# bowang-lab/gcn-drug-repurposing

Measured on AMD Instinct MI355X. Metric: gcn_spmm_edges_per_s, higher is better.
Workload: dtype f32; 1 GPU; whole_graph stand-in (value = 2.001e+10 edges/s counts every SpMM at nnz as the reference executes it; value_executed = 1.69e+10 counts the entries the kernels visited): N=29960, nnz(A_hat)=988028, d=128, L=2, B=2048, 15 steps/epoch; full train step (fwd+gss_loss+bwd+Adam), 6 SpMMs/step counted at nnz each (algorithmic; the top layer's first backward SpMM visits only entries whose neighbour is a b; parallelism=single; nodes relabelled hub-first

## Files before the change

gcn-drug-repurposing_amd/_lib.py:

```python
from __future__ import annotations

import ctypes as C
import os
import subprocess

_HERE = os.path.dirname(os.path.abspath(__file__))
LIB_PATH = os.path.join(_HERE, "libgssgcn.so")
CSRC = os.path.join(_HERE, "csrc")
ABI_VERSION = 21

_lib = None


class GssError(RuntimeError):
    pass


class PlanDesc(C.Structure):
    _fields_ = [("n", C.c_int32), ("d", C.c_int32), ("num_layers", C.c_int32), ("max_batch", C.c_int32),
                ("layer_decay", C.c_float), ("alpha", C.c_float), ("lr", C.c_float), ("beta1", C.c_float),
                ("beta2", C.c_float), ("eps", C.c_float), ("cache_layer1", C.c_int32), ("pipeline_layer1", C.c_int32),
                ("node_map", C.c_void_p)]


# ... 91 lines not shown
    "gss_edgelist_bad_line": (_I64, [_P]),
    "gss_edgelist_copy": (C.c_int, [_P, _P, _P, _P]),
    "gss_edgelist_close": (None, [_P]),
    "gss_plan_create": (C.c_int, [C.POINTER(_P), C.POINTER(PlanDesc), _P, _P, C.POINTER(PlanIO)]),
    "gss_plan_create_sharded": (C.c_int, [C.POINTER(_P), C.POINTER(PlanDesc), C.POINTER(ShardDesc), _P, _P, _P, C.POINTER(PlanIO)]),
    "gss_plan_gather_embeddings": (C.c_int, [_P, _P, _P]),
    "gss_plan_destroy": (None, [_P]),
    "gss_plan_forward": (C.c_int, [_P, _P]),
    "gss_plan_loss_backward": (C.c_int, [_P, _P, _I32, _F, _P]),
    "gss_plan_backward": (C.c_int, [_P, _P, _I32, _P, _P]),
    "gss_plan_adam": (C.c_int, [_P, _P]),
    "gss_plan_step": (C.c_int, [_P, _P, _I32, _F, _P]),
    "gss_plan_step_lazy": (C.c_int, [_P, _P, _I32, _F, _P]),
    "gss_plan_activation": (_P, [_P, C.c_int, C.c_int]),
    "gss_plan_device_bytes": (_SZ, [_P]),
    "gss_plan_check_guards": (C.c_int, [_P]),
    "gss_plan_lazy_halo_rows": (C.c_int, [_P, C.POINTER(_I64)]),
    "gss_plan_comm_stats": (C.c_int, [_P, C.POINTER(_I64)]),
    "gss_plan_sync_stats": (C.c_int, [_P, C.POINTER(_I64)]),
    "gss_comm_local_mode": (C.c_int, [_P, _I32]),
    "gss_comm_local_log": (C.c_int, [_P, C.POINTER(_I64), _I32, C.POINTER(_I32)]),
    "gss_plan_set_step": (None, [_P, _I32]),
    "gss_plan_adam_buffer": (_P, [_P, _I32, _I32]),
    "gss_plan_get_step": (_I32, [_P]),
    "gss_plan_profile": (C.c_int, [_P, C.c_int]),
    "gss_plan_profile_read": (C.c_int, [_P, C.POINTER(C.c_double), C.POINTER(C.c_int64), _P]),
    "gss_debug_set_option": (C.c_int, [C.c_char_p, C.c_int]),
    "gss_plan_debug_set_option": (C.c_int, [_P, C.c_char_p, C.c_int]),
    "gss_memcpy_d2d": (C.c_int, [_P, _P, _SZ, _P]),
    "gss_ppr_create": (C.c_int, [C.POINTER(_P), C.POINTER(PprDesc)]),
# ... 26 lines not shown
    "gss_rank_metrics_workspace_bytes": (_SZ, [_I32, _I32]),
    "gss_rank_metrics_rows": (C.c_int, [_I32, _I32, _P, _I64, _P, _P, _I32, _P, _P, _P, _P, _P, _P, _P, _SZ, _P]),
    "gss_profile_dist": (C.c_int, [_I32, _P, _I64, _I32, _P, _I32, _P, _I32, _P, _I64, _P]),
    "gss_profile_dist_pairs_workspace_bytes": (_SZ, [_I32, _I32]),
    "gss_profile_dist_pairs": (C.c_int, [_I32, _P, _I64, _I32, _P, _P, _I32, _P, _P, _SZ, _P]),
    "gss_profile_rank_workspace_bytes": (_SZ, [_I32, _I32]),
    "gss_profile_rank": (C.c_int, [_I32, _P, _I64, _I32, _P, _P, _I64, _P, _SZ, _P]),
    "gss_profile_topk_workspace_bytes": (_SZ, [_I32, _I32, _I32, _I32]),
    "gss_profile_topk": (C.c_int, [_I32, _P, _I64, _I32, _P, _I32, _P, _I32, _P, _P, _P, _P, _SZ, _P]),
    "gss_topk_overlap": (C.c_int, [_I32, _I32, _I32, _P, _P, _I32, _P, _P, _P, _P]),
    "gss_embedding_scores": (C.c_int, [_I32, _I32, _P, _I64, _I32, _P, _I32, _P, _I32, _P, _I64, _P]),
    "gss_spmm_bwd1_sparse_ex": (C.c_int, [_P, _I32, _P, _P, _P, _P, _P, _P, _P, _P, _P, _P, _I32, _P, _P]),
    "gss_spmm_bwd2_sparse_res": (C.c_int, [_P, _I32, _P, _P, _P, _F, _P, _P, _P, _P, _P, _P, _I32, _P]),
    "gss_spmm_filtered": (C.c_int, [_P, _I32, _P, _P, _P, _P, _P, _P, _P, _P, _P]),
    "gss_mark_rows_and_neighbours": (C.c_int, [_P, _P, _I32, _P, _P]),
    "gss_batch_bits": (C.c_int, [_P, _I32, _P, _I32, _P]),
    "gss_bits_fill": (C.c_int, [_P, _I64, _I64, _P]),
    "gss_loss_workspace_bytes_parts": (_SZ, [_I32, _I32, _I32]),
    "gss_loss_step": (C.c_int, [_I32, _I32, _F, _F, _P, _P, _P, _P, _P, _P, _P, _P, _F, _P, _P, _P, _P, _P, _P, _I32, _P, _P, _P, C.POINTER(_I32)]),
    "gss_loss_slab_sweep": (C.c_int, [_I32, _I32, _F, _F, _P, _I32, _I32, _P, _P, _P]),
    "gss_loss_gather_rows": (C.c_int, [_I32, _P, _P, _P, _I32, _P, C.POINTER(_P), _P]),
    "gss_loss_gather_rows_mapped": (C.c_int, [_I32, _P, _P, _P, _I32, _I32, _P, _P, _P, _P, _I32, _P, C.POINTER(_P), _P]),
    "gss_loss_gather_batch": (C.c_int, [_I32, _P, _P, _P, _P, _P, _I32, _I32, _P, _P, _P, _P, _P, _I32, _P, _P]),
    "gss_dense_fwd_rows": (C.c_int, [_I32, _I32, _P, _P, _P, _P, _P, _P, _P, _F, _P, _P, _P, _I32, _P]),
    "gss_dense_fwd_first": (C.c_int, [_I32, _I32, _P, _P, _P, _P]),
    "gss_dense_fwd_split_available": (C.c_int, [_I32, _I32]),
    "gss_dense_fwd_norm": (C.c_int, [_I32, _I32, _P, _P, _P, _P, _P, _P, _P, _F, _P, _P, _P, _P, _P, _P, _I32, _P]),
    "gss_rownorm_fwd_rows": (C.c_int, [_I32, _I32, _P, _P, _P, _P, _P]),
    "gss_wgrad_slices": (C.c_int, [_I32, _I32]),
    "gss_wgrad_slices_max": (C.c_int, [_I32, _I32]),
# ... 103 lines not shown
```

gcn-drug-repurposing_amd/csrc/ops.h:

```cpp
#pragma once
#include <memory>
#include <vector>

#include "common.h"

struct gss_giant_rows;

struct gss_csr {
  int32_t n_rows = 0, n_cols = 0;
  int64_t nnz = 0;
  const int32_t *rowptr = nullptr, *col = nullptr;
  const float *val = nullptr;
  int32_t n_long = 0;
  int32_t *d_long_rows = nullptr;
  int32_t max_row = 0;
  int32_t hot_own = -1, hot_halo0 = 0, hot_halo1 = 0;
  int32_t seg_edges = 32;
  std::vector<int32_t> h_rowptr;
  bool by_items = false;
  std::vector<int32_t> item_row, item_first, item_len;
  struct Cache {
    int32_t *segs[5] = {};
    int32_t seg_blocks[5] = {};
    std::unique_ptr<gss_giant_rows> giant;
// ... 43 lines not shown
};
int csr_segments(const gss_csr *a, int gpw_log2, const int4 **out, int *n_blocks);
struct LiveHint {
  int64_t prev;
  explicit LiveHint(int64_t rows);
  ~LiveHint();
  LiveHint(const LiveHint &) = delete;
  LiveHint &operator=(const LiveHint &) = delete;
};
int spmm_fwd(const gss_csr *a, int32_t d, const float *x, float *y, const float *h, float *m, void *stream,
             const int32_t *row_pos = nullptr,
             const uint32_t *row_bits = nullptr,
             const float *y_in = nullptr,
             const uint32_t *gather_bits = nullptr,
             const BatchPrep *prep = nullptr);
int mark_rows_and_neighbours(const gss_csr *a, const int32_t *rows, int32_t b, uint32_t *bits, void *stream);
int spmm_bwd1(const gss_csr *at, int32_t d, const float *g_am, const float *g_ax, const float *x_in, const float *ax,
              float *u, float *t, void *stream, const float *y_in = nullptr);
int spmm_bwd2(const gss_csr *at, int32_t d, const float *u, const float *t, const float *p, float c, const float *res,
              float *dp, float *gx_out, void *stream, const float *y_in = nullptr,
              int32_t own_row_limit = 0);
int dense_fwd(int32_t n, int32_t d, const float *ax, const float *am, const float *w1, const float *b1, const float *w2,
              const float *b2, const float *p_prev, float decay, float *p, float *x_next, void *stream,
              const int32_t *row_list = nullptr,
              bool acc_in_p = false);
bool dense_fwd_split_available(int32_t n, int32_t d);
bool dense_fwd_split_auto(int32_t n, int32_t d);
int dense_fwd_first(int32_t n, int32_t d, const float *ax, const float *w1, float *acc, void *stream);
bool dense_fwd_norm_available(int32_t d);
int dense_fwd_norm(int32_t n, int32_t d, const float *ax, const float *am, const float *w1, const float *b1, const float *w2,
// ... 107 lines not shown
```

gcn-drug-repurposing_amd/csrc/plan.hip:

```cpp
#include <algorithm>
#include <chrono>
#include <thread>
#include <vector>

#include "ops.h"

struct gss_plan {
  gss::Knobs knobs;
  gss_plan_desc desc;
  const gss_csr *a, *at;
  const float *x;
  float *w1, *b1, *w2, *b2;
  char *slab;
  size_t slab_bytes;
  std::vector<float *> ax, am, p, xin;
  float *m_tmp, *x_last, *emb, *inv_den;
  float *g_ax, *g_am, *u, *t, *dp, *gx[2];
  float *de_b, *dx_b, *dp_b, *gax_b, *gam_b;
  int32_t *pos;
  uint32_t *posbits;
  std::vector<size_t> guard_off;
  uint32_t *needbits;
  bool needbits_valid = false;
  uint32_t *nzbits;
  float *w1t, *w2t;
  float *grad[4];
  float *adam_m[4], *adam_v[4];
  float *loss;
  void *loss_ws, *wgrad_ws;
  int32_t step;
  bool layer1_valid;
  hipStream_t side;
  hipEvent_t ev_main_ready, ev_side_done;
  std::vector<hipEvent_t> ev_split_go, ev_split_done;
  float *ax0[2], *am0[2], *m_side;
  int cur0;
  bool prefetched;
  bool wt_valid;
  int wg_total;
  bool prof_on;
  std::vector<hipEvent_t> ev;
  std::vector<int> ev_cls;
  size_t ev_used;
  double prof_ms[GSS_PROF_CLASSES];
  int64_t prof_cnt[GSS_PROF_CLASSES];
  gss_comm *comm;
  int P, rank;
  int lo;
  std::vector<int64_t> h_bounds;
  struct Halo {
    int64_t n_halo = 0, n_send = 0;
    std::vector<int64_t> recv_off, send_off;
    const int32_t *d_send_rows = nullptr;
  } halo_a, halo_t;
  size_t rows_a, rows_t;
  const int32_t *gid2op_t;
  float *sendbuf;
// ... 44 lines not shown
  gss_plan *p;
  hipStream_t st;
  size_t slot;
  bool on;
  ProfScope(gss_plan *plan, int cls, void *stream) : p(plan), st(as_stream(stream)), slot(0), on(plan->prof_on) {
    if (!on) return;
    if (p->ev_used * 2 + 2 > p->ev.size()) {
      hipEvent_t a, b;
      if (hipEventCreate(&a) != hipSuccess || hipEventCreate(&b) != hipSuccess) {
        on = false;
        return;
      }
      p->ev.push_back(a);
      p->ev.push_back(b);
      p->ev_cls.push_back(cls);
    }
    slot = p->ev_used++;
    p->ev_cls[slot] = cls;
    (void)hipEventRecord(p->ev[2 * slot], st);
  }
  ~ProfScope() {
    if (on) (void)hipEventRecord(p->ev[2 * slot + 1], st);
  }
};
#define PROF(cls) ProfScope prof_scope_##__LINE__(p, cls, stream)

constexpr size_t kGuardBytes = 256;
constexpr int kGuardByte = 0xA5;
struct Carver {
  size_t off = 0;
  char *base = nullptr;
  std::vector<size_t> *guards = nullptr;
  template <typename T>
  T *take(size_t count) {
    off = (off + 255) / 256 * 256;
    T *p = base ? reinterpret_cast<T *>(base + off) : nullptr;
    off += sizeof(T) * count;
    off = (off + 255) / 256 * 256;
    if (guards) guards->push_back(off);
    off += kGuardBytes;
// ... 222 lines not shown
  p->a = a;
  p->at = at;
  p->x = io->x;
  p->w1 = io->w1;
  p->b1 = io->b1;
  p->w2 = io->w2;
  p->b2 = io->b2;
  p->emb = io->emb;
  p->loss = io->loss;
  p->grad[0] = io->gw1;
  p->grad[1] = io->gb1;
  p->grad[2] = io->gw2;
  p->grad[3] = io->gb2;
  p->step = 0;
  p->layer1_valid = false;
  p->wt_valid = false;

  p->prof_on = false;
  p->ev_used = 0;
  for (int k = 0; k < GSS_PROF_CLASSES; ++k) {
    p->prof_ms[k] = 0.0;
    p->prof_cnt[k] = 0;
  }
  {
    const int knob = K().lazy_halo, knob_u = K().lazy_halo_u;
    const bool rccl = comm && comm->device_transport();
    p->lz.on = P > 1 && desc->num_layers > 1 && (knob == 1 || (knob < 0 && n_global >= 262144 && !rccl));
    p->lzt.on = p->lz.on && spmm_sparse_available() && (knob_u == 1 || (knob_u < 0 && (knob == 1 || !rccl)));
    auto word_offsets = [&](gss_plan::LazyHalo &z, const gss_plan::Halo &h) {
      if (!z.on) return;
// ... 335 lines not shown

int plan_forward_impl(gss_plan *p, void *stream, const int32_t *lazy_rows = nullptr, int32_t lazy_b = 0) {
  if (p) p->needbits_valid = false;
  GSS_REQUIRE(p, "plan_forward: null plan");
  const gss_plan_desc &D = p->desc;
  const int L = D.num_layers;
  bool have_l0 = false;
  if (p->prefetched) {
    GSS_HIP(hipStreamWaitEvent(as_stream(stream), p->ev_side_done, 0));
    p->prefetched = false;
    p->cur0 ^= 1;
    p->ax[0] = p->ax0[p->cur0];
    p->am[0] = p->am0[p->cur0];
    have_l0 = true;
  }
  for (int l = 0; l < L; ++l) {
    float *xl = p->xin[l];
    const bool cached = (l == 0 && ((D.cache_layer1 && p->layer1_valid) || have_l0));
    bool split_l = false;
    if (!cached) {
      if (l == 0)
        if (int rc = plan_x0(p, stream)) return rc;
      const bool split_a = p->a_own != nullptr;
      float *m = l == 0 ? p->m0op : p->m_tmp;
      const bool lazy_l = lazy_rows && l == L - 1;
      const bool needed_only = lazy_l && p->P > 1 && p->lz.on;
      if (needed_only) {
        if (!p->lz_pending)
          if (int rc = plan_lazy_requests_begin(p, lazy_rows, lazy_b, stream)) return rc;
        if (int rc = plan_lazy_requests_end(p, stream)) return rc;
      }
      if (lazy_l && p->needbits) {
        PROF(GSS_PROF_ELEMENTWISE);
        GSS_HIP(hipMemsetAsync(p->needbits, 0, sizeof(uint32_t) * (p->rows_a / 32 + 1), as_stream(stream)));
        if (int rc = mark_rows_and_neighbours(p->a, lazy_rows, lazy_b, p->needbits, stream)) return rc;
        if (needed_only)
          if (int rc = bits_set_list(p->needbits, p->lz.send_list, p->lz.h_cnt[p->P], stream)) return rc;
        p->needbits_valid = p->P == 1 || needed_only;
      }
      const int64_t deg_a = p->a->n_rows > 0 ? p->a->nnz / p->a->n_rows : 0;
      LiveHint hint_nb(lazy_l ? (int64_t)lazy_b * (1 + deg_a) : 0);
      {
        const uint32_t *rbits = (lazy_l && p->needbits) ? p->needbits : nullptr;
        auto full = [&]() {
          PROF(GSS_PROF_SPMM_FWD_HAD);
          const BatchPrep *prep = p->prep_pending;
          p->prep_pending = nullptr;
          return spmm_fwd(p->a, D.d, xl, p->ax[l], xl, m, stream, nullptr, rbits, nullptr, nullptr, prep);
        };
        if (l == 0 || (l == 1 && p->recompute)) {
          if (int rc = full()) return rc;
        } else {
          auto own = [&]() {
            PROF(GSS_PROF_SPMM_FWD_HAD);
            return spmm_fwd(p->a_own, D.d, xl, p->ax[l], nullptr, nullptr, stream, nullptr, rbits);
          };
          auto rest = [&]() {
            PROF(GSS_PROF_SPMM_FWD_HAD);
            return spmm_fwd(p->a_halo, D.d, xl, p->ax[l], xl, m, stream, nullptr, rbits, p->ax[l]);
          };
          if (int rc = plan_hop(p, p->halo_a, split_a, xl, stream, full, own, rest)) return rc;
        }
// ... 1 lines not shown
      split_l = (int)p->ev_split_go.size() == L && !lazy_l && p->P == 1 && !D.pipeline_layer1 && dense_fwd_split_available(D.n, D.d) &&
                (K().proj_split == 1 || (K().proj_split < 0 && dense_fwd_split_auto(D.n, D.d)));
      if (split_l) {
        GSS_HIP(hipEventRecord(p->ev_split_go[l], as_stream(stream)));
        GSS_HIP(hipStreamWaitEvent(p->side, p->ev_split_go[l], 0));
        {
          ProfScope prof_first(p, GSS_PROF_DENSE_FWD, p->side);
          if (int rc = dense_fwd_first(D.n, D.d, p->ax[l], p->w1, p->p[l], p->side)) return rc;
        }
        GSS_HIP(hipEventRecord(p->ev_split_done[l], p->side));
      }
      {
        const int32_t *rpos = lazy_l ? p->pos : nullptr;
        LiveHint hint_b(lazy_l ? (int64_t)lazy_b : 0);
        auto full = [&]() {
          PROF(GSS_PROF_SPMM_FWD);
          return spmm_fwd(p->a, D.d, m, p->am[l], nullptr, nullptr, stream, rpos);
        };
        if (l == 0 && p->m0_ready) {
          if (int rc = full()) return rc;
        } else {
          auto own = [&]() {
            PROF(GSS_PROF_SPMM_FWD);
            return spmm_fwd(p->a_own, D.d, m, p->am[l], nullptr, nullptr, stream, rpos);
          };
          auto rest = [&]() {
            PROF(GSS_PROF_SPMM_FWD);
            return spmm_fwd(p->a_halo, D.d, m, p->am[l], nullptr, nullptr, stream, rpos, nullptr, p->am[l]);
          };
          if (int rc = plan_hop(p, p->halo_a, split_a, m, stream, full, own, rest, needed_only ? lazy_rows : nullptr, lazy_b)) return rc;
          if (l == 0) p->m0_ready = true;
// ... 365 lines not shown
  if (p->ev_ready) (void)hipEventDestroy(p->ev_ready);
  if (p->ev_halo) (void)hipEventDestroy(p->ev_halo);
  if (p->ev_main_ready) (void)hipEventDestroy(p->ev_main_ready);
  if (p->ev_side_done) (void)hipEventDestroy(p->ev_side_done);
  for (hipEvent_t e : p->ev_split_go) (void)hipEventDestroy(e);
  for (hipEvent_t e : p->ev_split_done) (void)hipEventDestroy(e);
  if (p->lz.h_cnt) (void)hipHostFree(p->lz.h_cnt);
  if (p->lzt.h_cnt) (void)hipHostFree(p->lzt.h_cnt);
  if (p->slab) (void)hipFree(p->slab);
  delete p;
}

int gss_plan_debug_set_option(gss_plan *p, const char *name, int value) {
  GSS_REQUIRE(p && name, "plan_debug_set_option: null argument");
  static const char *const kLive[] = {"gemm_variant", "spmm_slices", "spmm_pin", "gemm_ws", "spmm_list_blocks", "proj_split"};
  bool ok = false;
  for (const char *k : kLive) ok = ok || strcmp(k, name) == 0;
  GSS_REQUIRE(ok, "plan_debug_set_option: only kernel-selection knobs can change on a live plan");
  return gss::set_knob(p->knobs, name, value);
}

int gss_plan_forward(gss_plan *p, void *stream) {
  KnobScope knob_scope(p ? &p->knobs : nullptr);
  if (p) p->wt_valid = false;
  return plan_forward_impl(p, stream);
}
int gss_plan_loss_backward(gss_plan *p, const int32_t *idx, int32_t b, float beta, void *stream) {
  KnobScope knob_scope(p ? &p->knobs : nullptr);
  if (p) p->wt_valid = false;
  BatchView bv{};
// ... 22 lines not shown

int gss_plan_step_lazy(gss_plan *p, const int32_t *idx, int32_t b, float beta, void *stream) {
  KnobScope knob_scope(p ? &p->knobs : nullptr);
  GSS_REQUIRE(p, "plan_step_lazy: null plan");
  const gss_plan_desc &D = p->desc;
  const bool can = D.num_layers > 1 && spmm_sparse_available() && !D.pipeline_layer1 && p->pos;
  return plan_step_impl(p, idx, b, beta, stream, can);
}

static int plan_step_impl(gss_plan *p, const int32_t *idx, int32_t b, float beta, void *stream, bool lazy) {
  GSS_REQUIRE(p, "plan_step: null plan");
  const bool pipe = p->desc.pipeline_layer1 && p->side && !p->prof_on && !p->desc.cache_layer1;
  const gss_plan_desc &D0 = p->desc;
  const bool mapped0 = plan_batch_mapped(p);
  const bool sparse0 = D0.num_layers > 1 && spmm_sparse_available() && p->pos;
  const bool l0_runs = !(D0.cache_layer1 && p->layer1_valid) && !p->prefetched;
  const bool host_prep = p->P == 1 && sparse0 && K().prep_side != 0 && idx && b >= 1 && b <= D0.max_batch &&
                         (l0_runs || !(lazy && p->needbits));
  BatchPrep prep{idx, b, D0.node_map, p->lo, D0.n, p->gid2op_t, mapped0 ? p->rloc : nullptr, mapped0 ? p->pid : nullptr, p->keep, p->pos, p->rlist};
  bool prepared = lazy;
  if (host_prep) {
    p->prep_pending = &prep;
    prepared = true;
    p->eb_scatter_b = (!lazy && dense_fwd_norm_available(D0.d)) ? b : 0;
  }
  if (lazy) {
    GSS_REQUIRE(idx && b >= 1 && b <= p->desc.max_batch, "plan_step_lazy: batch %d out of [1, %d]", b, p->desc.max_batch);
    const bool mapped = plan_batch_mapped(p);
    if (!host_prep) {
      PROF(GSS_PROF_ELEMENTWISE);
      if (int rc = batch_prepare(idx, b, p->desc.node_map, p->lo, p->desc.n, p->gid2op_t, mapped ? p->rloc : nullptr, mapped ? p->pid : nullptr,
// ... 72 lines not shown
      rc = fail(GSS_EHIP, "plan_gather_embeddings: copy of shard %d failed", r);
  }
  (void)hipFreeAsync(stage, st);
  return rc;
}

const float *gss_plan_activation(const gss_plan *p, int layer, int which) {
  if (!p || layer < 0 || layer >= p->desc.num_layers) return nullptr;
  if (which == 5) return p->u;
  if (which == 6) return p->t;
  if (which == 7) return reinterpret_cast<const float *>(p->nzbits);
  if (which == 8) return p->gab;
  return which == 0 ? p->ax[layer] : which == 1 ? p->am[layer] : which == 2 ? p->p[layer] : which == 3 ? p->dp : which == 4 ? p->dp_b : nullptr;
}
size_t gss_plan_device_bytes(const gss_plan *p) { return p ? p->slab_bytes : 0; }

int gss_plan_lazy_halo_rows(const gss_plan *p, int64_t *out6) {
  GSS_REQUIRE(p && out6, "plan_lazy_halo_rows: null argument");
  out6[0] = p->lz.on ? p->lz.last_recv : -1;
  out6[1] = p->lz.on ? p->lz.last_send : -1;
  out6[2] = p->halo_a.n_halo;
  out6[3] = p->lzt.on ? p->lzt.last_recv : -1;
  out6[4] = p->lzt.on ? p->lzt.last_send : -1;
  out6[5] = p->halo_t.n_halo;
  return GSS_OK;
}

int gss_plan_comm_stats(gss_plan *p, int64_t *out3) {
  GSS_REQUIRE(p && out3, "plan_comm_stats: null argument");
  for (int k = 0; k < 3; ++k) {
// ... 36 lines not shown
}
int32_t gss_plan_get_step(const gss_plan *p) { return p ? p->step : 0; }
int gss_plan_profile(gss_plan *p, int enable) {
  GSS_REQUIRE(p, "plan_profile: null plan");
  p->prof_on = enable != 0;
  return GSS_OK;
}

int gss_plan_profile_read(gss_plan *p, double *ms_out, int64_t *count_out, void *stream) {
  GSS_REQUIRE(p && ms_out && count_out, "plan_profile_read: null argument");
  GSS_HIP(hipStreamSynchronize(as_stream(stream)));
  for (size_t k = 0; k < p->ev_used; ++k) {
    float ms = 0.f;
    GSS_HIP(hipEventElapsedTime(&ms, p->ev[2 * k], p->ev[2 * k + 1]));
    p->prof_ms[p->ev_cls[k]] += ms;
    p->prof_cnt[p->ev_cls[k]] += 1;
  }
  p->ev_used = 0;
  for (int k = 0; k < GSS_PROF_CLASSES; ++k) {
    ms_out[k] = p->prof_ms[k];
    count_out[k] = p->prof_cnt[k];
    p->prof_ms[k] = 0.0;
    p->prof_cnt[k] = 0;
  }
  return GSS_OK;
}

int gss_memcpy_d2d(void *dst, const void *src, size_t bytes, void *stream) {
  GSS_REQUIRE(dst && src, "memcpy_d2d: null pointer");
  GSS_HIP(hipMemcpyAsync(dst, src, bytes, hipMemcpyDeviceToDevice, as_stream(stream)));
  return GSS_OK;
// ... 3 lines not shown
```

gcn-drug-repurposing_amd/csrc/spmm.hip:

```cpp
#include <algorithm>
#include <vector>

#include "ops.h"
#include "segments.h"

namespace gss {

constexpr int kLongRow = 512;
constexpr int kRowsPerBlock = 16;
constexpr int kLongThreads = 1024;

enum SpmmMode { SPMM_PLAIN = 0, SPMM_FWD1 = 1, SPMM_BWD1 = 2, SPMM_BWD2 = 3, SPMM_BWD1S = 4, SPMM_BWD2S = 5 };

struct SpmmEpi {
  const float *a0, *a1, *a2;
  float *o0, *o1;
  float c;
  const int32_t *pos;
  const int32_t *pos_row;
  const uint32_t *posbits;
  uint32_t *nzbits_out;
  int skip_zero_rows;
  const float *y_in;
  const uint32_t *gather_bits;
// ... 435 lines not shown
      piece_live |= !is_zero4(t[v]);
    }
    bool tz = row_t_zero<MODE>(ep, row);
    if (MODE == SPMM_BWD1S) tz = row_mark_nonzero<MODE>(ep, row, piece_live, gmask);
#pragma unroll
    for (int v = 0; v < VPL; ++v) {
      const int f4 = li + v * 64;
      if (f4 >= d4) continue;
      const long coff = compact_off<MODE>(ep, row, rs4, slice_f4 + f4);
      row_epilogue<MODE>(ep, ((size_t)row * rs4 + slice_f4 + f4) * 4, t[v], coff, tz);
    }
  }
}


template <int MODE, int LPR_LOG2, int VPL, bool NARROW>
__global__ __launch_bounds__(kBalThreads) void spmm_balanced_kernel(CsrView a, const int4 *__restrict__ segs, int d4,
                                                                   const float *__restrict__ x, SpmmEpi ep, int rowstride_f, int pin_ns, int3 hot) {
  extern __shared__ __attribute__((aligned(16))) char smem[];
  float4 *part = reinterpret_cast<float4 *>(smem);
  const bool has_prep = MODE == SPMM_FWD1 && ep.prep.idx != nullptr;
  const int bx = (int)blockIdx.x - (has_prep ? 1 : 0);
  const int sblk = pin_ns > 0 ? bx / pin_ns : bx;
  const int sidx = pin_ns > 0 ? bx % pin_ns : (int)blockIdx.y;
  if (has_prep && blockIdx.x == 0) {
    if (blockIdx.y == 0) {
      const BatchPrep &q = ep.prep;
      for (int i = threadIdx.x; i < q.b; i += kBalThreads) {
        const int id = q.node_map ? q.node_map[q.idx[i]] : q.idx[i];
        const int rel = id - q.lo;
        const bool mine = rel >= 0 && rel < q.nl;
        const int op = q.gid2op ? q.gid2op[id] : (mine ? rel : -1);
        if (q.rloc) q.rloc[i] = min(max(rel, 0), max(q.nl - 1, 0));
        if (q.pid) q.pid[i] = op;
        if (q.keep) q.keep[i] = mine ? 1.f : 0.f;
        if (q.rlist) q.rlist[i] = mine ? rel : -1;
        if (op >= 0) q.pos[op] = i;
      }
    }
    return;
  }
  spmm_balanced_block<MODE, LPR_LOG2, VPL, NARROW>(a, segs, d4, x, ep, rowstride_f, sblk, sidx, hot, part);
}

static thread_local int64_t t_live_hint = 0;
}
gss::LiveHint::LiveHint(int64_t rows) : prev(gss::t_live_hint) { gss::t_live_hint = rows; }
gss::LiveHint::~LiveHint() { gss::t_live_hint = prev; }
namespace gss {
struct LiveFilter {
  const int32_t *pos;
  const uint32_t *bits;
  const int32_t *row_alias;
};
__global__ __launch_bounds__(256) void live_blocks_kernel(const int4 *__restrict__ segs, int nblk, int groups_per_block, LiveFilter f,
                                                          int32_t *__restrict__ out) {
  const int lane = threadIdx.x & 63;
// ... 72 lines not shown
  } else {
    nblk = build_segments(a->h_rowptr.data(), a->n_rows, kBalWaves, gpw_log2, a->seg_edges, segs);
  }
  const size_t bytes = segs.size() * sizeof(int32_t);
  if (bytes) {
    GSS_HIP(hipMalloc((void **)&c.segs[gpw_log2], bytes));
    GSS_HIP(hipMemcpy(c.segs[gpw_log2], segs.data(), bytes, hipMemcpyHostToDevice));
  }
  c.seg_blocks[gpw_log2] = nblk;
  *out = (const int4 *)c.segs[gpw_log2];
  *n_blocks = nblk;
  return GSS_OK;
}


template <int MODE, int LPR_LOG2, int VPL>
static int launch_balanced_t(const gss_csr *a, int d4_slice, int nslices, bool pin, const float *x, const SpmmEpi &ep_in, hipStream_t st) {
  const int4 *segs = nullptr;
  int nblk = 0;
  if (int rc = csr_segments(a, 6 - LPR_LOG2, &segs, &nblk)) return rc;
  if (nblk == 0 && !(MODE == SPMM_FWD1 && ep_in.prep.idx)) return GSS_OK;
  CsrView v{a->rowptr, a->col, a->val, a->n_rows};
  const size_t lds = (size_t)kBalWaves * d4_slice * sizeof(float4);
  SpmmEpi ep = ep_in;
  const bool prep = MODE == SPMM_FWD1 && ep.prep.idx != nullptr;
  ep.prep_block = 0;
  const int extra = prep ? 1 : 0;
  int3 hot = make_int3(a->hot_own, a->hot_halo0, a->hot_halo1);
  if (K().spmm_hot >= 0) hot = K().spmm_hot > 0 ? make_int3(K().spmm_hot, 0, 0) : make_int3(-1, 0, 0);
  if ((double)a->n_cols * d4_slice * nslices * 16.0 < 256.0 * 1024 * 1024 && K().spmm_hot < 0) hot = make_int3(-1, 0, 0);
  const bool narrow = (double)a->n_cols * d4_slice * nslices * 16.0 < 4.0e9 && a->n_cols < (1 << 24) && hot.x < 0;
  if constexpr (MODE == SPMM_PLAIN || MODE == SPMM_FWD1 || MODE == SPMM_BWD1S) {
// ... 11 lines not shown
      hipLaunchKernelGGL(live_blocks_kernel, dim3(ceil_div(nblk, 4)), dim3(256), 0, st, segs, nblk, kBalWaves * (64 >> LPR_LOG2), f, live);
      GSS_LAUNCH_CHECK("live_blocks_kernel");
      int gx = std::min(nblk, kListWorkgroups);
      if (pin) gx = std::max(nslices, gx / nslices * nslices);
      const dim3 grid = pin ? dim3(gx) : dim3(gx, nslices);
      if (narrow)
        hipLaunchKernelGGL((spmm_balanced_list_kernel<MODE, LPR_LOG2, VPL, true>), grid, dim3(kBalThreads), lds, st, v, segs, d4_slice, x, ep,
                           d4_slice * nslices * 4, pin ? nslices : 0, make_int3(-1, 0, 0), (const int32_t *)live);
      else
        hipLaunchKernelGGL((spmm_balanced_list_kernel<MODE, LPR_LOG2, VPL, false>), grid, dim3(kBalThreads), lds, st, v, segs, d4_slice, x, ep,
                           d4_slice * nslices * 4, pin ? nslices : 0, hot, (const int32_t *)live);
      GSS_LAUNCH_CHECK("spmm_balanced_list_kernel");
      return GSS_OK;
    }
  }
  if (narrow)
    hipLaunchKernelGGL((spmm_balanced_kernel<MODE, LPR_LOG2, VPL, true>), pin ? dim3(nblk * nslices + extra) : dim3(nblk + extra, nslices), dim3(kBalThreads),
                       lds, st, v, segs, d4_slice, x, ep, d4_slice * nslices * 4, pin ? nslices : 0, make_int3(-1, 0, 0));
  else
    hipLaunchKernelGGL((spmm_balanced_kernel<MODE, LPR_LOG2, VPL, false>), pin ? dim3(nblk * nslices + extra) : dim3(nblk + extra, nslices), dim3(kBalThreads),
                       lds, st, v, segs, d4_slice, x, ep, d4_slice * nslices * 4, pin ? nslices : 0, hot);
  GSS_LAUNCH_CHECK("spmm_balanced_kernel");
  return GSS_OK;
}

template <int MODE>
static int launch_balanced(const gss_csr *a, int d4, const float *x, const SpmmEpi &ep, hipStream_t st) {
  int ns = K().spmm_slices;
  bool pin = K().spmm_pin != 0;
  if (ns == 0) {
    const double table = 16.0 * d4 * (double)a->n_cols;
    ns = 1;
    pin = false;
    if (d4 >= 32 && d4 % 16 == 0 && table > 8.0 * 1024 * 1024) {
      ns = d4 / 16 > 8 ? 8 : d4 / 16;
      while (d4 % ns != 0) --ns;
      pin = table <= 64.0 * 1024 * 1024;
    }
  }
  if (ns < 1 || d4 % ns != 0 || (d4 / ns) < 4 || MODE == SPMM_BWD1S) ns = 1;
  pin = pin && ns > 1;
  const int ds = d4 / ns;
  if (ds <= 4) return launch_balanced_t<MODE, 2, 1>(a, ds, ns, pin, x, ep, st);
  if (ds <= 8) return launch_balanced_t<MODE, 3, 1>(a, ds, ns, pin, x, ep, st);
  if (ds <= 16) return launch_balanced_t<MODE, 4, 1>(a, ds, ns, pin, x, ep, st);
  if (ds <= 32) return launch_balanced_t<MODE, 5, 1>(a, ds, ns, pin, x, ep, st);
  if (ds <= 64) return launch_balanced_t<MODE, 6, 1>(a, ds, ns, pin, x, ep, st);
  if (ds <= 128) return launch_balanced_t<MODE, 6, 2>(a, ds, ns, pin, x, ep, st);
  return launch_balanced_t<MODE, 6, 4>(a, ds, ns, pin, x, ep, st);
}

}

struct gss_giant_rows {
  int32_t n_giant = 0, n_chunks = 0;
  gss_csr chunks, shortv, finish;
  int32_t *d_chunk_row = nullptr, *d_fin_col = nullptr;
  float *d_fin_val = nullptr;
  ~gss_giant_rows() {
    if (d_chunk_row) (void)hipFree(d_chunk_row);
    if (d_fin_col) (void)hipFree(d_fin_col);
    if (d_fin_val) (void)hipFree(d_fin_val);
  }
};
// ... 153 lines not shown
  GSS_REQUIRE(!gather_bits || !m, "spmm: a gather filter goes with the plain product only");
  if (m) {
    GSS_REQUIRE(h, "spmm: m given without h");
    SpmmEpi ep{h, nullptr, nullptr, y, m, 0.f, nullptr, nullptr, row_bits};
    ep.y_in = y_in;
    if (prep) ep.prep = *prep;
    return launch_spmm<SPMM_FWD1>(a, d, x, ep, stream);
  }
  SpmmEpi ep{nullptr, nullptr, nullptr, y, nullptr, 0.f, row_pos, nullptr, nullptr};
  ep.y_in = y_in;
  ep.gather_bits = gather_bits;
  ep.rowbits = row_bits;
  return launch_spmm<SPMM_PLAIN>(a, d, x, ep, stream);
}

int spmm_bwd1(const gss_csr *at, int32_t d, const float *g_am, const float *g_ax, const float *x_in, const float *ax,
              float *u, float *t, void *stream, const float *y_in) {
  GSS_REQUIRE(g_am && g_ax && x_in && ax && u && t, "spmm_bwd1: null operand");
  GSS_REQUIRE(!y_in || K().spmm_variant == 2, "spmm_bwd1: a two-pass product needs the balanced SpMM (spmm_variant 2)");
  SpmmEpi ep{g_ax, x_in, ax, u, t, 0.f, nullptr, nullptr, nullptr, nullptr};
  ep.y_in = y_in;
  return launch_spmm<SPMM_BWD1>(at, d, g_am, ep, stream);
}

int spmm_bwd1_sparse(const gss_csr *at, int32_t d, const float *g_am_b, const float *g_ax_b, const int32_t *pos,
                     const int32_t *pos_row, const float *x_in, const float *ax, float *u, float *t, void *stream, const uint32_t *posbits,
                     uint32_t *nzbits_out, int skip_zero_rows, const uint32_t *live_rows) {
  GSS_REQUIRE(g_am_b && g_ax_b && pos && pos_row && x_in && ax && u && t, "spmm_bwd1_sparse: null operand");
  GSS_REQUIRE(K().spmm_variant == 2, "spmm_bwd1_sparse needs the balanced SpMM (spmm_variant 2)");
  GSS_REQUIRE(!skip_zero_rows || nzbits_out, "spmm_bwd1_sparse: skipping the zero rows needs the bitmap that records them");
// ... 251 lines not shown
                            uint32_t *nzbits_out, int32_t skip_zero_rows, const uint32_t *live_rows, void *stream) {
  GSS_REQUIRE(at, "gss_spmm_bwd1_sparse_ex: null handle");
  return spmm_bwd1_sparse(at, d, g_am_b, g_ax_b, pos_col, pos_row, x_in, ax, u, t, stream, posbits, nzbits_out, skip_zero_rows, live_rows);
}
int gss_spmm_bwd2_sparse_res(const gss_csr *at, int32_t d, const float *u, const float *t, const float *p, float c, const float *res_b,
                             const int32_t *pos_row, float *dp, float *gx_out, const uint32_t *nzbits, const float *y_in,
                             int32_t pos_row_limit, void *stream) {
  GSS_REQUIRE(at, "gss_spmm_bwd2_sparse_res: null handle");
  return spmm_bwd2_sparse_res(at, d, u, t, p, c, res_b, pos_row, dp, gx_out, stream, nzbits, y_in, pos_row_limit);
}
int gss_spmm_filtered(const gss_csr *a, int32_t d, const float *x, float *y, const float *h, float *m, const int32_t *row_pos,
                      const uint32_t *row_bits, const float *y_in, const uint32_t *gather_bits, void *stream) {
  GSS_REQUIRE(a && x && y, "gss_spmm_filtered: null operand");
  return spmm_fwd(a, d, x, y, h, m, stream, row_pos, row_bits, y_in, gather_bits);
}
int gss_mark_rows_and_neighbours(const gss_csr *a, const int32_t *rows, int32_t b, uint32_t *bits, void *stream) {
  return mark_rows_and_neighbours(a, rows, b, bits, stream);
}
}
```

include/gssgcn.h:

```cpp
#ifndef GSSGCN_H
#define GSSGCN_H

#include <stddef.h>
#include <stdint.h>

#ifdef __cplusplus
extern "C" {
#endif

#define GSS_ABI_VERSION 21

#define GSS_OK 0
#define GSS_EINVAL (-22)
#define GSS_ENOMEM (-12)
#define GSS_EHIP (-5)
#define GSS_ENOTCONV (-34)
#define GSS_ECOMM (-104)
#define GSS_ETIMEOUT (-110)

typedef struct gss_csr gss_csr;
typedef struct gss_plan gss_plan;
typedef struct gss_comm gss_comm;

int gss_abi_version(void);
const char *gss_source_hash(const char *file);
int gss_plan_debug_set_option(gss_plan *plan, const char *name, int value);
const char *gss_last_error(void);

int gss_normalize_adj(int32_t n, const int32_t *rowptr, const int32_t *col, const double *val,
                      float *val_out, double *rowsum_out, void *stream);

int gss_rowsum_dinv(int32_t n, const int32_t *rowptr, const double *val, double *dinv_out, double *rowsum_out, void *stream);
int gss_scale_adj_shard(int32_t n, int32_t row0, const int32_t *rowptr, const int32_t *col, const double *val, const double *dinv_global,
                        int32_t transposed, float *val_out, void *stream);
int gss_rowsum_check(int32_t n, const double *rowsum, int64_t *h_count_out, int32_t *h_first_out, void *stream);

int gss_csr_create(gss_csr **out, int32_t n_rows, int32_t n_cols, int64_t nnz, const int32_t *h_rowptr,
                   const int32_t *d_rowptr, const int32_t *d_col, const float *d_val);
void gss_csr_destroy(gss_csr *a);
int gss_csr_set_hot(gss_csr *a, int32_t own_hot, int32_t halo_begin, int32_t halo_end);
int gss_csr_giant_rows(const gss_csr *a, int32_t *n_rows_out, int32_t *n_chunks_out);
// ... 281 lines not shown
};
int gss_plan_profile(gss_plan *p, int enable);
int gss_plan_profile_read(gss_plan *p, double *ms_out, int64_t *count_out, void *stream);
int gss_debug_set_option(const char *name, int value);
int gss_memcpy_d2d(void *dst, const void *src, size_t bytes, void *stream);

int gss_spmm_bwd1_sparse_ex(const gss_csr *at, int32_t d, const float *g_am_b, const float *g_ax_b, const int32_t *pos_col,
                            const int32_t *pos_row, const float *x_in, const float *ax, float *u, float *t, const uint32_t *posbits,
                            uint32_t *nzbits_out, int32_t skip_zero_rows, const uint32_t *live_rows, void *stream);
int gss_spmm_bwd2_sparse_res(const gss_csr *at, int32_t d, const float *u, const float *t, const float *p, float c, const float *res_b,
                             const int32_t *pos_row, float *dp, float *gx_out, const uint32_t *nzbits, const float *y_in,
                             int32_t pos_row_limit, void *stream);
int gss_spmm_filtered(const gss_csr *a, int32_t d, const float *x, float *y, const float *h, float *m, const int32_t *row_pos,
                      const uint32_t *row_bits, const float *y_in, const uint32_t *gather_bits, void *stream);
int gss_mark_rows_and_neighbours(const gss_csr *a, const int32_t *rows, int32_t b, uint32_t *bits, void *stream);
int gss_batch_bits(const int32_t *ids, int32_t b, uint32_t *bits, int32_t set, void *stream);
int gss_bits_fill(uint32_t *bits, int64_t first, int64_t last, void *stream);

size_t gss_loss_workspace_bytes_parts(int32_t b, int32_t d, int32_t parts);
int gss_loss_step(int32_t d, int32_t b, float beta, float alpha, float *loss_out, const float *e_b, const int32_t *rows,
                  const int32_t *pos_ids, int32_t *pos_set, const float *keep, const float *inv_den, const float *p, float c, float *dx_b,
                  float *dp_b, const float *w1t, const float *w2t, float *gax_b, float *gam_b, int32_t dgrad_all, const float *de_x,
                  void *ws, void *stream, int32_t *dgrad_done);
int gss_loss_slab_sweep(int32_t d, int32_t b, float beta, float alpha, const float *e_b, int32_t slab_rank, int32_t slab_parts, void *ws,
                        float *de_x, void *stream);
int gss_loss_gather_rows(int32_t d, const float *e, const int32_t *rows, const float *keep, int32_t b, void *ws, float **e_b_out,
                         void *stream);
int gss_loss_gather_rows_mapped(int32_t d, const float *e, const int32_t *idx, const int32_t *node_map, int32_t lo, int32_t nl,
                                const int32_t *gid2op, int32_t *pid, int32_t *rloc, float *keep, int32_t b, void *ws, float **e_b_out,
                                void *stream);
// ... 35 lines not shown
```

Baseline: 19.99 billion edges/s.

## Pair next step's layer-0 forward SpMMs with layer-1 SpMMs in one launch

```diff
diff --git a/gcn-drug-repurposing_amd/_lib.py b/gcn-drug-repurposing_amd/_lib.py
--- a/gcn-drug-repurposing_amd/_lib.py
+++ b/gcn-drug-repurposing_amd/_lib.py
@@ -7,7 +7,7 @@
 _HERE = os.path.dirname(os.path.abspath(__file__))
 LIB_PATH = os.path.join(_HERE, "libgssgcn.so")
 CSRC = os.path.join(_HERE, "csrc")
-ABI_VERSION = 21
+ABI_VERSION = 22
 
 _lib = None
 
@@ -129,6 +129,7 @@
     "gss_plan_step_lazy": (C.c_int, [_P, _P, _I32, _F, _P]),
     "gss_plan_activation": (_P, [_P, C.c_int, C.c_int]),
     "gss_plan_device_bytes": (_SZ, [_P]),
+    "gss_plan_l1_ahead": (C.c_int, [_P]),
     "gss_plan_check_guards": (C.c_int, [_P]),
     "gss_plan_lazy_halo_rows": (C.c_int, [_P, C.POINTER(_I64)]),
     "gss_plan_comm_stats": (C.c_int, [_P, C.POINTER(_I64)]),
@@ -185,6 +186,7 @@
     "gss_spmm_bwd2_sparse_res": (C.c_int, [_P, _I32, _P, _P, _P, _F, _P, _P, _P, _P, _P, _P, _I32, _P]),
     "gss_spmm_filtered": (C.c_int, [_P, _I32, _P, _P, _P, _P, _P, _P, _P, _P, _P]),
     "gss_mark_rows_and_neighbours": (C.c_int, [_P, _P, _I32, _P, _P]),
+    "gss_spmm_fwd_pair": (C.c_int, [_P, _I32, _P, _P, _P, _P, _P, _P, _P, _P, _P, _I32, _P, _P, _P, _P, _P, _P]),
     "gss_batch_bits": (C.c_int, [_P, _I32, _P, _I32, _P]),
     "gss_bits_fill": (C.c_int, [_P, _I64, _I64, _P]),
     "gss_loss_workspace_bytes_parts": (_SZ, [_I32, _I32, _I32]),
diff --git a/gcn-drug-repurposing_amd/csrc/ops.h b/gcn-drug-repurposing_amd/csrc/ops.h
--- a/gcn-drug-repurposing_amd/csrc/ops.h
+++ b/gcn-drug-repurposing_amd/csrc/ops.h
@@ -81,6 +81,14 @@
              const float *y_in = nullptr,
              const uint32_t *gather_bits = nullptr,
              const BatchPrep *prep = nullptr);
+struct SpmmFwdArgs {
+  const float *x;
+  float *y;
+  const float *h;
+  float *m;
+};
+int spmm_fwd_pair(const gss_csr *a, int32_t d, const SpmmFwdArgs &p0, const SpmmFwdArgs &p1, void *stream, const BatchPrep *prep = nullptr,
+                  int *paired_out = nullptr);
 int mark_rows_and_neighbours(const gss_csr *a, const int32_t *rows, int32_t b, uint32_t *bits, void *stream);
 int spmm_bwd1(const gss_csr *at, int32_t d, const float *g_am, const float *g_ax, const float *x_in, const float *ax,
               float *u, float *t, void *stream, const float *y_in = nullptr);
diff --git a/gcn-drug-repurposing_amd/csrc/plan.hip b/gcn-drug-repurposing_amd/csrc/plan.hip
--- a/gcn-drug-repurposing_amd/csrc/plan.hip
+++ b/gcn-drug-repurposing_amd/csrc/plan.hip
@@ -30,6 +30,8 @@
   void *loss_ws, *wgrad_ws;
   int32_t step;
   bool layer1_valid;
+  bool l1_ahead;
+  int l1_ahead_opt;
   hipStream_t side;
   hipEvent_t ev_main_ready, ev_side_done;
   std::vector<hipEvent_t> ev_split_go, ev_split_done;
@@ -41,6 +43,7 @@
   bool prof_on;
   std::vector<hipEvent_t> ev;
   std::vector<int> ev_cls;
+  std::vector<int> ev_n;
   size_t ev_used;
   double prof_ms[GSS_PROF_CLASSES];
   int64_t prof_cnt[GSS_PROF_CLASSES];
@@ -115,16 +118,23 @@
       p->ev.push_back(a);
       p->ev.push_back(b);
       p->ev_cls.push_back(cls);
+      p->ev_n.push_back(1);
     }
     slot = p->ev_used++;
     p->ev_cls[slot] = cls;
+    p->ev_n[slot] = 1;
     (void)hipEventRecord(p->ev[2 * slot], st);
   }
   ~ProfScope() {
     if (on) (void)hipEventRecord(p->ev[2 * slot + 1], st);
   }
+  void products(int n) {
+    if (on) p->ev_n[slot] = n;
+  }
 };
 #define PROF(cls) ProfScope prof_scope_##__LINE__(p, cls, stream)
+
+constexpr bool l1_ahead_auto() { return true; }
 
 constexpr size_t kGuardBytes = 256;
 constexpr int kGuardByte = 0xA5;
@@ -377,6 +387,8 @@
   p->grad[3] = io->gb2;
   p->step = 0;
   p->layer1_valid = false;
+  p->l1_ahead = false;
+  p->l1_ahead_opt = -1;
   p->wt_valid = false;
 
   p->prof_on = false;
@@ -742,6 +754,13 @@
     p->am[0] = p->am0[p->cur0];
     have_l0 = true;
   }
+  if (p->l1_ahead) {
+    p->l1_ahead = false;
+    have_l0 = true;
+  }
+  const bool ahead = p->P == 1 && L >= 2 && !D.cache_layer1 && !D.pipeline_layer1 && !lazy_rows && D.n > 0 &&
+                     (p->l1_ahead_opt == 1 || (p->l1_ahead_opt < 0 && l1_ahead_auto()));
+  float *l1_m = p->dp;
   for (int l = 0; l < L; ++l) {
     float *xl = p->xin[l];
     const bool cached = (l == 0 && ((D.cache_layer1 && p->layer1_valid) || have_l0));
@@ -771,9 +790,13 @@
       {
         const uint32_t *rbits = (lazy_l && p->needbits) ? p->needbits : nullptr;
         auto full = [&]() {
-          PROF(GSS_PROF_SPMM_FWD_HAD);
+          ProfScope prof(p, GSS_PROF_SPMM_FWD_HAD, stream);
           const BatchPrep *prep = p->prep_pending;
           p->prep_pending = nullptr;
+          if (ahead && l == 1) {
+            prof.products(2);
+            return spmm_fwd_pair(p->a, D.d, SpmmFwdArgs{xl, p->ax[l], xl, m}, SpmmFwdArgs{p->xin[0], p->ax[0], p->xin[0], l1_m}, stream, prep);
+          }
           return spmm_fwd(p->a, D.d, xl, p->ax[l], xl, m, stream, nullptr, rbits, nullptr, nullptr, prep);
         };
         if (l == 0 || (l == 1 && p->recompute)) {
@@ -805,7 +828,13 @@
         const int32_t *rpos = lazy_l ? p->pos : nullptr;
         LiveHint hint_b(lazy_l ? (int64_t)lazy_b : 0);
         auto full = [&]() {
-          PROF(GSS_PROF_SPMM_FWD);
+          ProfScope prof(p, GSS_PROF_SPMM_FWD, stream);
+          if (ahead && l == 1) {
+            prof.products(2);
+            const int rc = spmm_fwd_pair(p->a, D.d, SpmmFwdArgs{m, p->am[l], nullptr, nullptr}, SpmmFwdArgs{l1_m, p->am[0], nullptr, nullptr}, stream);
+            p->l1_ahead = rc == GSS_OK;
+            return rc;
+          }
           return spmm_fwd(p->a, D.d, m, p->am[l], nullptr, nullptr, stream, rpos);
         };
         if (l == 0 && p->m0_ready) {
@@ -1201,6 +1230,11 @@
 int gss_plan_debug_set_option(gss_plan *p, const char *name, int value) {
   GSS_REQUIRE(p && name, "plan_debug_set_option: null argument");
   static const char *const kLive[] = {"gemm_variant", "spmm_slices", "spmm_pin", "gemm_ws", "spmm_list_blocks", "proj_split"};
+  if (strcmp(name, "l1_ahead") == 0) {
+    GSS_REQUIRE(value >= -1 && value <= 1, "l1_ahead must be -1 (automatic), 0 or 1");
+    p->l1_ahead_opt = value;
+    return GSS_OK;
+  }
   bool ok = false;
   for (const char *k : kLive) ok = ok || strcmp(k, name) == 0;
   GSS_REQUIRE(ok, "plan_debug_set_option: only kernel-selection knobs can change on a live plan");
@@ -1253,7 +1287,7 @@
   const gss_plan_desc &D0 = p->desc;
   const bool mapped0 = plan_batch_mapped(p);
   const bool sparse0 = D0.num_layers > 1 && spmm_sparse_available() && p->pos;
-  const bool l0_runs = !(D0.cache_layer1 && p->layer1_valid) && !p->prefetched;
+  const bool l0_runs = !(D0.cache_layer1 && p->layer1_valid) && !p->prefetched && !p->l1_ahead;
   const bool host_prep = p->P == 1 && sparse0 && K().prep_side != 0 && idx && b >= 1 && b <= D0.max_batch &&
                          (l0_runs || !(lazy && p->needbits));
   BatchPrep prep{idx, b, D0.node_map, p->lo, D0.n, p->gid2op_t, mapped0 ? p->rloc : nullptr, mapped0 ? p->pid : nullptr, p->keep, p->pos, p->rlist};
@@ -1356,6 +1390,7 @@
   return which == 0 ? p->ax[layer] : which == 1 ? p->am[layer] : which == 2 ? p->p[layer] : which == 3 ? p->dp : which == 4 ? p->dp_b : nullptr;
 }
 size_t gss_plan_device_bytes(const gss_plan *p) { return p ? p->slab_bytes : 0; }
+int gss_plan_l1_ahead(const gss_plan *p) { return p && p->l1_ahead ? 1 : 0; }
 
 int gss_plan_lazy_halo_rows(const gss_plan *p, int64_t *out6) {
   GSS_REQUIRE(p && out6, "plan_lazy_halo_rows: null argument");
@@ -1422,7 +1457,7 @@
     float ms = 0.f;
     GSS_HIP(hipEventElapsedTime(&ms, p->ev[2 * k], p->ev[2 * k + 1]));
     p->prof_ms[p->ev_cls[k]] += ms;
-    p->prof_cnt[p->ev_cls[k]] += 1;
+    p->prof_cnt[p->ev_cls[k]] += p->ev_n[k];
   }
   p->ev_used = 0;
   for (int k = 0; k < GSS_PROF_CLASSES; ++k) {
diff --git a/gcn-drug-repurposing_amd/csrc/spmm.hip b/gcn-drug-repurposing_amd/csrc/spmm.hip
--- a/gcn-drug-repurposing_amd/csrc/spmm.hip
+++ b/gcn-drug-repurposing_amd/csrc/spmm.hip
@@ -473,6 +473,20 @@
 }
 
 
+__device__ __forceinline__ void batch_prep_block(const BatchPrep &q) {
+  for (int i = threadIdx.x; i < q.b; i += kBalThreads) {
+    const int id = q.node_map ? q.node_map[q.idx[i]] : q.idx[i];
+    const int rel = id - q.lo;
+    const bool mine = rel >= 0 && rel < q.nl;
+    const int op = q.gid2op ? q.gid2op[id] : (mine ? rel : -1);
+    if (q.rloc) q.rloc[i] = min(max(rel, 0), max(q.nl - 1, 0));
+    if (q.pid) q.pid[i] = op;
+    if (q.keep) q.keep[i] = mine ? 1.f : 0.f;
+    if (q.rlist) q.rlist[i] = mine ? rel : -1;
+    if (op >= 0) q.pos[op] = i;
+  }
+}
+
 template <int MODE, int LPR_LOG2, int VPL, bool NARROW>
 __global__ __launch_bounds__(kBalThreads) void spmm_balanced_kernel(CsrView a, const int4 *__restrict__ segs, int d4,
                                                                    const float *__restrict__ x, SpmmEpi ep, int rowstride_f, int pin_ns, int3 hot) {
@@ -483,23 +497,31 @@
   const int sblk = pin_ns > 0 ? bx / pin_ns : bx;
   const int sidx = pin_ns > 0 ? bx % pin_ns : (int)blockIdx.y;
   if (has_prep && blockIdx.x == 0) {
-    if (blockIdx.y == 0) {
-      const BatchPrep &q = ep.prep;
-      for (int i = threadIdx.x; i < q.b; i += kBalThreads) {
-        const int id = q.node_map ? q.node_map[q.idx[i]] : q.idx[i];
-        const int rel = id - q.lo;
-        const bool mine = rel >= 0 && rel < q.nl;
-        const int op = q.gid2op ? q.gid2op[id] : (mine ? rel : -1);
-        if (q.rloc) q.rloc[i] = min(max(rel, 0), max(q.nl - 1, 0));
-        if (q.pid) q.pid[i] = op;
-        if (q.keep) q.keep[i] = mine ? 1.f : 0.f;
-        if (q.rlist) q.rlist[i] = mine ? rel : -1;
-        if (op >= 0) q.pos[op] = i;
-      }
-    }
+    if (blockIdx.y == 0) batch_prep_block(ep.prep);
     return;
   }
   spmm_balanced_block<MODE, LPR_LOG2, VPL, NARROW>(a, segs, d4, x, ep, rowstride_f, sblk, sidx, hot, part);
+}
+
+template <int MODE, int LPR_LOG2, int VPL, bool NARROW>
+__global__ __launch_bounds__(kBalThreads) void spmm_balanced_pair_kernel(CsrView a, const int4 *__restrict__ segs, int d4, const float *__restrict__ x0,
+                                                                        SpmmEpi ep0, const float *__restrict__ x1, SpmmEpi ep1, int rowstride_f,
+                                                                        int pin_ns, int3 hot, int half) {
+  static_assert(MODE == SPMM_FWD1 || MODE == SPMM_PLAIN, "only the forward products are paired");
+  extern __shared__ __attribute__((aligned(16))) char smem[];
+  float4 *part = reinterpret_cast<float4 *>(smem);
+  const bool has_prep = MODE == SPMM_FWD1 && ep0.prep.idx != nullptr;
+  if (has_prep && blockIdx.x == 0) {
+    if (blockIdx.y == 0) batch_prep_block(ep0.prep);
+    return;
+  }
+  int bx = (int)blockIdx.x - (has_prep ? 1 : 0);
+  const bool second = bx >= half;
+  if (second) bx -= half;
+  const int sblk = pin_ns > 0 ? bx / pin_ns : bx;
+  const int sidx = pin_ns > 0 ? bx % pin_ns : (int)blockIdx.y;
+  const SpmmEpi &ep = second ? ep1 : ep0;
+  spmm_balanced_block<MODE, LPR_LOG2, VPL, NARROW>(a, segs, d4, second ? x1 : x0, ep, rowstride_f, sblk, sidx, hot, part);
 }
 
 static thread_local int64_t t_live_hint = 0;
@@ -602,8 +624,14 @@
 }
 
 
+struct SpmmSecond {
+  const float *x;
+  SpmmEpi ep;
+};
+
 template <int MODE, int LPR_LOG2, int VPL>
-static int launch_balanced_t(const gss_csr *a, int d4_slice, int nslices, bool pin, const float *x, const SpmmEpi &ep_in, hipStream_t st) {
+static int launch_balanced_t(const gss_csr *a, int d4_slice, int nslices, bool pin, const float *x, const SpmmEpi &ep_in, hipStream_t st,
+                             const SpmmSecond *second = nullptr) {
   const int4 *segs = nullptr;
   int nblk = 0;
   if (int rc = csr_segments(a, 6 - LPR_LOG2, &segs, &nblk)) return rc;
@@ -645,6 +673,20 @@
       return GSS_OK;
     }
   }
+  if constexpr (MODE == SPMM_PLAIN || MODE == SPMM_FWD1) {
+    if (second) {
+      const int half = pin ? nblk * nslices : nblk;
+      const dim3 grid = pin ? dim3(2 * half + extra) : dim3(2 * half + extra, nslices);
+      if (narrow)
+        hipLaunchKernelGGL((spmm_balanced_pair_kernel<MODE, LPR_LOG2, VPL, true>), grid, dim3(kBalThreads), lds, st, v, segs, d4_slice, x, ep, second->x,
+                           second->ep, d4_slice * nslices * 4, pin ? nslices : 0, make_int3(-1, 0, 0), half);
+      else
+        hipLaunchKernelGGL((spmm_balanced_pair_kernel<MODE, LPR_LOG2, VPL, false>), grid, dim3(kBalThreads), lds, st, v, segs, d4_slice, x, ep, second->x,
+                           second->ep, d4_slice * nslices * 4, pin ? nslices : 0, hot, half);
+      GSS_LAUNCH_CHECK("spmm_balanced_pair_kernel");
+      return GSS_OK;
+    }
+  }
   if (narrow)
     hipLaunchKernelGGL((spmm_balanced_kernel<MODE, LPR_LOG2, VPL, true>), pin ? dim3(nblk * nslices + extra) : dim3(nblk + extra, nslices), dim3(kBalThreads),
                        lds, st, v, segs, d4_slice, x, ep, d4_slice * nslices * 4, pin ? nslices : 0, make_int3(-1, 0, 0));
@@ -656,7 +698,7 @@
 }
 
 template <int MODE>
-static int launch_balanced(const gss_csr *a, int d4, const float *x, const SpmmEpi &ep, hipStream_t st) {
+static int launch_balanced(const gss_csr *a, int d4, const float *x, const SpmmEpi &ep, hipStream_t st, const SpmmSecond *second = nullptr) {
   int ns = K().spmm_slices;
   bool pin = K().spmm_pin != 0;
   if (ns == 0) {
@@ -672,13 +714,13 @@
   if (ns < 1 || d4 % ns != 0 || (d4 / ns) < 4 || MODE == SPMM_BWD1S) ns = 1;
   pin = pin && ns > 1;
   const int ds = d4 / ns;
-  if (ds <= 4) return launch_balanced_t<MODE, 2, 1>(a, ds, ns, pin, x, ep, st);
-  if (ds <= 8) return launch_balanced_t<MODE, 3, 1>(a, ds, ns, pin, x, ep, st);
-  if (ds <= 16) return launch_balanced_t<MODE, 4, 1>(a, ds, ns, pin, x, ep, st);
-  if (ds <= 32) return launch_balanced_t<MODE, 5, 1>(a, ds, ns, pin, x, ep, st);
-  if (ds <= 64) return launch_balanced_t<MODE, 6, 1>(a, ds, ns, pin, x, ep, st);
-  if (ds <= 128) return launch_balanced_t<MODE, 6, 2>(a, ds, ns, pin, x, ep, st);
-  return launch_balanced_t<MODE, 6, 4>(a, ds, ns, pin, x, ep, st);
+  if (ds <= 4) return launch_balanced_t<MODE, 2, 1>(a, ds, ns, pin, x, ep, st, second);
+  if (ds <= 8) return launch_balanced_t<MODE, 3, 1>(a, ds, ns, pin, x, ep, st, second);
+  if (ds <= 16) return launch_balanced_t<MODE, 4, 1>(a, ds, ns, pin, x, ep, st, second);
+  if (ds <= 32) return launch_balanced_t<MODE, 5, 1>(a, ds, ns, pin, x, ep, st, second);
+  if (ds <= 64) return launch_balanced_t<MODE, 6, 1>(a, ds, ns, pin, x, ep, st, second);
+  if (ds <= 128) return launch_balanced_t<MODE, 6, 2>(a, ds, ns, pin, x, ep, st, second);
+  return launch_balanced_t<MODE, 6, 4>(a, ds, ns, pin, x, ep, st, second);
 }
 
 }
@@ -862,6 +904,40 @@
   return launch_spmm<SPMM_PLAIN>(a, d, x, ep, stream);
 }
 
+int spmm_fwd_pair(const gss_csr *a, int32_t d, const SpmmFwdArgs &p0, const SpmmFwdArgs &p1, void *stream, const BatchPrep *prep, int *paired_out) {
+  if (paired_out) *paired_out = 0;
+  if (int rc = check_d(d)) return rc;
+  GSS_REQUIRE(a && p0.x && p0.y && p1.x && p1.y, "spmm_fwd_pair: null operand");
+  GSS_REQUIRE((p0.m != nullptr) == (p1.m != nullptr), "spmm_fwd_pair: both products Hadamard-fused or both plain");
+  GSS_REQUIRE((!p0.m || p0.h) && (!p1.m || p1.h), "spmm_fwd_pair: m given without h");
+  bool pair = K().spmm_variant == 2 && a->n_rows > 0 && a->nnz > 0;
+  if (pair) {
+    gss_giant_rows *g = nullptr;
+    if (int rc = csr_giant_rows(a, &g)) return rc;
+    pair = g == nullptr;
+  }
+  if (!pair) {
+    if (int rc = spmm_fwd(a, d, p0.x, p0.y, p0.h, p0.m, stream, nullptr, nullptr, nullptr, nullptr, prep)) return rc;
+    return spmm_fwd(a, d, p1.x, p1.y, p1.h, p1.m, stream);
+  }
+  GSS_REQUIRE(!prep || (p0.m && prep->idx && prep->pos && prep->b > 0), "spmm_fwd_pair: the batch-preparation side job goes with the Hadamard-fused product");
+  hipStream_t st = as_stream(stream);
+  SpmmSecond second{p1.x, SpmmEpi{}};
+  int rc;
+  if (p0.m) {
+    SpmmEpi ep{p0.h, nullptr, nullptr, p0.y, p0.m, 0.f, nullptr, nullptr, nullptr};
+    if (prep) ep.prep = *prep;
+    second.ep = SpmmEpi{p1.h, nullptr, nullptr, p1.y, p1.m, 0.f, nullptr, nullptr, nullptr};
+    rc = launch_balanced<SPMM_FWD1>(a, d / 4, p0.x, ep, st, &second);
+  } else {
+    SpmmEpi ep{nullptr, nullptr, nullptr, p0.y, nullptr, 0.f, nullptr, nullptr, nullptr};
+    second.ep = SpmmEpi{nullptr, nullptr, nullptr, p1.y, nullptr, 0.f, nullptr, nullptr, nullptr};
+    rc = launch_balanced<SPMM_PLAIN>(a, d / 4, p0.x, ep, st, &second);
+  }
+  if (rc == GSS_OK && paired_out) *paired_out = 1;
+  return rc;
+}
+
 int spmm_bwd1(const gss_csr *at, int32_t d, const float *g_am, const float *g_ax, const float *x_in, const float *ax,
               float *u, float *t, void *stream, const float *y_in) {
   GSS_REQUIRE(g_am && g_ax && x_in && ax && u && t, "spmm_bwd1: null operand");
@@ -1143,6 +1219,16 @@
   GSS_REQUIRE(a && x && y, "gss_spmm_filtered: null operand");
   return spmm_fwd(a, d, x, y, h, m, stream, row_pos, row_bits, y_in, gather_bits);
 }
+int gss_spmm_fwd_pair(const gss_csr *a, int32_t d, const float *x0, float *y0, const float *h0, float *m0, const float *x1, float *y1,
+                      const float *h1, float *m1, const int32_t *prep_idx, int32_t prep_b, const int32_t *prep_node_map, int32_t *prep_rloc,
+                      int32_t *prep_pid, int32_t *prep_pos, int32_t *paired_out, void *stream) {
+  GSS_REQUIRE(a, "gss_spmm_fwd_pair: null handle");
+  const BatchPrep bp{prep_idx, prep_b, prep_node_map, 0, a->n_rows, nullptr, prep_rloc, prep_pid, nullptr, prep_pos, nullptr};
+  int paired = 0;
+  const int rc = spmm_fwd_pair(a, d, SpmmFwdArgs{x0, y0, h0, m0}, SpmmFwdArgs{x1, y1, h1, m1}, stream, prep_idx ? &bp : nullptr, &paired);
+  if (paired_out) *paired_out = paired;
+  return rc;
+}
 int gss_mark_rows_and_neighbours(const gss_csr *a, const int32_t *rows, int32_t b, uint32_t *bits, void *stream) {
   return mark_rows_and_neighbours(a, rows, b, bits, stream);
 }
diff --git a/include/gssgcn.h b/include/gssgcn.h
--- a/include/gssgcn.h
+++ b/include/gssgcn.h
@@ -8,7 +8,7 @@
 extern "C" {
 #endif
 
-#define GSS_ABI_VERSION 21
+#define GSS_ABI_VERSION 22
 
 #define GSS_OK 0
 #define GSS_EINVAL (-22)
@@ -25,6 +25,7 @@
 int gss_abi_version(void);
 const char *gss_source_hash(const char *file);
 int gss_plan_debug_set_option(gss_plan *plan, const char *name, int value);
+int gss_plan_l1_ahead(const gss_plan *plan);
 const char *gss_last_error(void);
 
 int gss_normalize_adj(int32_t n, const int32_t *rowptr, const int32_t *col, const double *val,
@@ -336,6 +337,9 @@
 int gss_spmm_filtered(const gss_csr *a, int32_t d, const float *x, float *y, const float *h, float *m, const int32_t *row_pos,
                       const uint32_t *row_bits, const float *y_in, const uint32_t *gather_bits, void *stream);
 int gss_mark_rows_and_neighbours(const gss_csr *a, const int32_t *rows, int32_t b, uint32_t *bits, void *stream);
+int gss_spmm_fwd_pair(const gss_csr *a, int32_t d, const float *x0, float *y0, const float *h0, float *m0, const float *x1, float *y1,
+                      const float *h1, float *m1, const int32_t *prep_idx, int32_t prep_b, const int32_t *prep_node_map, int32_t *prep_rloc,
+                      int32_t *prep_pid, int32_t *prep_pos, int32_t *paired_out, void *stream);
 int gss_batch_bits(const int32_t *ids, int32_t b, uint32_t *bits, int32_t set, void *stream);
 int gss_bits_fill(uint32_t *bits, int64_t first, int64_t last, void *stream);
 
```

After: 20.41 billion edges/s (median of 6 runs). +2.1%, better.
